# projecthorus/radiosonde_auto_rx

Measured on AMD Instinct MI355X. Metric: IQ Msamples/s (RS41 --IQ --lpIQ demod + framesync + ECC), concurrent real-time 2.4 Msps channels = value/2.4, higher is better.
Workload: dtype f32; 1 GPU; RS41 2.4 Msps cs16 IQ, rs41mod --ecc2 --IQ fq --lpIQ (BASELINE configs[1]) x 512 channels per GPU (per-GPU share of configs[4]), 1 s of signal per channel per step, input resident in HBM; channels_per_gpu=512, frames_decoded=507392, frames_ecc_ok=457842, frames_ecc_failed=49550, frames_repaired=200182, symbols_repaired=1815512

## Files before the change

radiosonde_auto_rx_amd/csrc/sonde_dev.h:

```cpp
#ifndef SONDE_DEV_H
#define SONDE_DEV_H
#include <hip/hip_runtime.h>
#include <stdint.h>
#include "../../include/sonde_hip.h"

struct MixDecArgs {
    const int16_t *iq;
    long long ch_stride;
    int n_ch, nblocks;
    int D, Q;
    int G;
    int wgs_per_ch;
    float wtab[64 * 8];
    const double *chan_f0;
    int lut_len;
    uint32_t lut_phase;
    const float2 *dc_avg;
    long long *dc_sums;
    const float2 *ptail_in;
    float2 *ptail_out;
    float2 *y;
    int ring_len;
    uint32_t m0;
    const float *wtab_g;
// ... 66 lines not shown
};

struct AudioChainArgs {
    const float *raw; float *fm, *bufs; const float *w;
    int n_ch, ring_len, n, taps; uint32_t m0;
};

struct SyncState {
    uint32_t s_in, k, mv_pos, mode;
    float mv; uint32_t inv;
    uint32_t pad[2];
};

struct WinItem {
    uint32_t pos;
    int32_t  state;
    int32_t  rc;
    float    mv; uint32_t mpos;
    uint32_t pad[3];
};
struct WinPlanArgs {
    const SyncState *state; WinItem *items;
    int n_ch, stride, W, K, L, delay; uint32_t frame_samples, avail;
    const uint32_t *epoch;
    uint32_t *work, *work_count; int round_parity;
};
struct WinFftArgs {
    const float *bufs; WinItem *items; const float2 *Fm, *tws;
    int n_ch, stride, W, K, L, ring_len;
    const uint32_t *work, *work_count; int round_parity;
    unsigned long long *prof;
    int small_wg;
    float2 *park;
};
#define SONDE_WFH_MAXGRID 768

struct CorrArgs {
    const float *bufs; float *corr; const float *match;
    const SyncState *state;
    const uint32_t *start;
    int delay; uint32_t frame_samples;
    uint32_t limit;
    int n_ch, ring_len, n, L; uint32_t m0;
    int ntypes, isps, nsym;
    const float *shapes;
    const int *sym_type;
    const float *sym_sign;
};

struct FrameRec {
    int32_t channel, len, nbytes; uint32_t mv_pos; float mv;
    int32_t ecc, ecc_done;
    uint8_t synd[48];
    uint8_t frame[520];
};

struct SyncArgs {
    const float *bufs, *corr; SyncState *state; FrameRec *frames; unsigned *frame_count; float *soft;
    float *soft1;
    const uint8_t *hdr, *hdr_bytes, *mask, *gf_exp, *gf_log;
    const uint4 *bitwin;
    const uint32_t *bitend;
    int n_ch, ring_len, max_frames; uint32_t avail;
    int K, L, delay, hdrlen, symhd, symlen, hdmax, bitofs, nbits; uint32_t frame_samples;
    float sps, thres, l_win;
    int rs41;
// ... 48 lines not shown
```

radiosonde_auto_rx_amd/csrc/sonde_engine.cpp:

```cpp
#include "../../include/sonde_hip.h"
#include "sonde_dev.h"
#include "sonde_host.h"
#include "sonde_scan_dev.h"
#include <algorithm>
#include <cmath>
#include <cstdio>
#include <cstring>
#include <map>
#include <string>
#include <vector>

using namespace sonde;

#define HIPCHK(x) do { hipError_t e_ = (x); if (e_ != hipSuccess) { fprintf(stderr, "libsonde_hip: %s failed: %s\n", #x, hipGetErrorString(e_)); return SONDE_E_NOGPU; } } while (0)

struct KernelStat { double ms = 0; int64_t n = 0; };
struct PendingEvt { hipEvent_t a, b; const char *name; };

struct sonde_engine {
    sonde_cfg_t cfg{};
    sonde_info_t info{};
    hipStream_t stream = nullptr;
    hipStream_t stream_b = nullptr;
    unsigned long long *d_wfprof = nullptr;
// ... 24 lines not shown
    float *d_wiq = nullptr, *d_wfm = nullptr, *d_match = nullptr;
    uint32_t corr_limit = 0;
    WinItem *d_win = nullptr; float2 *d_Fm = nullptr, *d_tws = nullptr; int win_W = 0;
    uint32_t *d_work = nullptr, *d_work_count = nullptr; int sync_rounds = 0;
    sonde_summary_t *d_summary = nullptr; uint32_t summary_base = 0;
    sonde_summary_t *d_summary_snap = nullptr;
    int corr_types = 0, corr_isps = 0; float *d_shapes = nullptr, *d_symsign = nullptr; int *d_symtype = nullptr;
    SyncState *d_state = nullptr; FrameRec *d_frames = nullptr; unsigned *d_fcount = nullptr; float *d_soft = nullptr, *d_soft1 = nullptr;
    uint4 *d_bitwin = nullptr; uint32_t *d_bitend = nullptr;
    uint8_t *d_consts = nullptr;
    int16_t *d_stage = nullptr; size_t stage_bytes = 0;
    bool ifiq = false;
    int opt_iq = 5; float match_sum = 0.f;
    std::vector<float> w_iq0; float *d_wiq0 = nullptr;
    float2 *d_yrot = nullptr; float *d_fmraw = nullptr, *d_corr2 = nullptr;
    AfcState *d_afc = nullptr; uint32_t *d_start = nullptr; unsigned *d_pending = nullptr, *h_pending = nullptr;
    double *d_dcsums_f = nullptr; float2 *d_zring = nullptr; float *d_taps_f = nullptr; uint32_t zmask = 0;
    hipEvent_t ev_copy = nullptr;
    int16_t *d_conv = nullptr;
    float2 *d_conv32 = nullptr; bool f32_path = false, conv32 = false;
    int ring_len = 0, max_frames = 0;
    uint64_t samples_in = 0;
    uint32_t m_out = 0;
    uint32_t dc_cnt = 0, dc_max = 0, dc_lim = 0;
    bool pcs = false; std::vector<uint32_t> pcs_cnt, pcs_max; uint32_t dc_max0 = 0;
    uint32_t *d_epoch_phase = nullptr, *d_pcs_cnt = nullptr, *d_pcs_max = nullptr; int32_t *d_pcs_since = nullptr;
    std::vector<float> last_soft, last_soft1; int last_n = 0;
    std::vector<uint8_t> last_frame;
    std::vector<char> m10_bits;
    bool overflow = false;
    bool in_call = false, ecc_listed = false;
    float2 *d_park = nullptr;
    bool small_tail = false;
    bool dev_ecc = true;
    long long host_ecc_frames = 0;
    bool m10_chk3 = false;
    std::vector<uint32_t> epoch; uint32_t *d_epoch = nullptr; int eof_ch = -1;
    bool prof = false, prof_skip = false; int prof_level = 2; std::map<std::string, KernelStat> stats; std::vector<PendingEvt> pend;
    std::vector<sonde_engine *> groups; std::vector<int32_t> grp_of_ch, row_of_ch; std::vector<std::vector<int32_t>> ch_of_grp; int32_t *d_in_row = nullptr;
    bool front_only = false; int64_t snap_calls = 0;
    sonde_engine *front = nullptr; int front_row = 0; int32_t *d_sum_map = nullptr; bool is_group = false;
    bool merged = false, borrowed_b = false;
};
struct CreateLink { bool is_group, front_only; int min_ring; hipStream_t shared_b; };

template <class T> static int dalloc(T **p, size_t n, bool zero = true) {
    HIPCHK(hipMalloc((void **)p, n * sizeof(T)));
    if (zero) HIPCHK(hipMemset(*p, 0, n * sizeof(T)));
    return 0;
}

static void prof_begin(sonde_engine *e, const char *name, hipStream_t s) {
    if (!e->prof || (e->prof_level == 1 && strcmp(name, "mix_decimate") != 0)) { e->prof_skip = true; return; }
    e->prof_skip = false;
    PendingEvt p; p.name = name;
    hipEventCreate(&p.a); hipEventCreate(&p.b);
    hipEventRecord(p.a, s);
    e->pend.push_back(p);
}
static void prof_end(sonde_engine *e, hipStream_t s) { if (e->prof && !e->prof_skip) hipEventRecord(e->pend.back().b, s); }
static void prof_collect(sonde_engine *e) {
    for (auto &p : e->pend) {
        float ms = 0; hipEventSynchronize(p.b); hipEventElapsedTime(&ms, p.a, p.b);
        auto &s = e->stats[p.name]; s.ms += ms; s.n += 1;
        hipEventDestroy(p.a); hipEventDestroy(p.b);
    }
// ... 289 lines not shown
        HIPCHK(hipMemcpy(e->d_chanf0, f0s.data(), f0s.size() * sizeof(double), hipMemcpyHostToDevice));
    }
    {
        static const bool no_fast = getenv("SONDE_MD_NOFAST") != nullptr;
        if (D == 50 && e->Q == 7 && !audio && cfg->bits != 32 && cfg->sonde_type != SONDE_FRONTEND && !cfg->opt_nolut && e->lut_len % D == 0 && !no_fast
            && cfg->input == SONDE_IN_IQ && !is_group) {
            e->etab_len = e->lut_len / D;
            if (dalloc(&e->d_etab, (size_t)C * e->etab_len, false) || dalloc(&e->d_dcavg_prev, C)) { sonde_engine_destroy(e); return SONDE_E_NOMEM; }
            sonde_launch_md_etable(e->d_chanf0, e->d_wtab, D, e->Q, e->etab_len, C, e->d_etab, nullptr);
            HIPCHK(hipDeviceSynchronize());
        }
    }
    int bad = 0;
    bad |= dalloc(&e->d_dcavg, C); bad |= dalloc(&e->d_dcsums, 2 * (size_t)C);
    bad |= dalloc(&e->d_ptail[0], (size_t)C * 64); bad |= dalloc(&e->d_ptail[1], (size_t)C * 64);
    if (audio) bad |= dalloc(&e->d_raw, (size_t)C * ring);
    else { if (!is_group) bad |= dalloc(&e->d_y, (size_t)C * ring); if (!front_only) bad |= dalloc(&e->d_ifiq, (size_t)C * ring); }
    if (!front_only) { bad |= dalloc(&e->d_fm, (size_t)C * ring); bad |= dalloc(&e->d_bufs, (size_t)C * ring); bad |= dalloc(&e->d_corr, (size_t)C * ring); }
    bad |= dalloc(&e->d_state, C); bad |= dalloc(&e->d_frames, e->max_frames); bad |= dalloc(&e->d_fcount, 1 + 4);
    if (cfg->keep_soft || cfg->sonde_type != SONDE_RS41) bad |= dalloc(&e->d_soft, (size_t)e->max_frames * e->nbits);
    if (cfg->keep_soft == 2) bad |= dalloc(&e->d_soft1, (size_t)e->max_frames * e->nbits);
    if (cfg->sonde_type == SONDE_DFM09) { bad |= dalloc(&e->d_dfm_out, (size_t)e->max_frames * 8); bad |= dalloc(&e->d_blk_done, 2); }
    if (cfg->sonde_type == SONDE_M10) { bad |= dalloc(&e->d_m10_out, (size_t)e->max_frames); bad |= dalloc(&e->d_blk_done, 2); bad |= dalloc(&e->d_m10_bits, (size_t)C * ((101 + 20) * 8 + 8)); }
    bad |= dalloc(&e->d_match, L, false);
    if (!e->w_iq.empty()) bad |= dalloc(&e->d_wiq, e->w_iq.size(), false);
    if (!e->w_fm.empty()) bad |= dalloc(&e->d_wfm, e->w_fm.size(), false);
    bad |= dalloc(&e->d_consts, 1024, true);
    if (bad) { sonde_engine_destroy(e); return SONDE_E_NOMEM; }
    HIPCHK(hipMemcpy(e->d_match, e->match.data(), L * sizeof(float), hipMemcpyHostToDevice));
    e->dev_ecc = getenv("SONDE_HOST_ECC") == nullptr;
    {
        const char *st = getenv("SONDE_SMALL_TAIL");
        e->small_tail = st && atoi(st) != 0;
    }
    {
        static const bool no_fft = getenv("SONDE_NO_FFTSYNC") != nullptr;
        if (!cfg->opt_dc && M == 8192 && K + L <= M && !no_fft) {
            std::vector<float> m(2 * (size_t)M, 0.f);
            for (int i = 0; i < L; i++) m[2 * (size_t)(L - 1 - i)] = e->match[i];
            ref_dft_8192(m);
            const std::vector<float> tw = ref_twiddle_table();
            e->win_W = 8;
            m.resize(4 * (size_t)M);
            for (int i = 0; i < M; i++) {
                int r = 0; for (int b = 0; b < 13; b++) if (i >> b & 1) r |= 1 << (12 - b);
                m[2 * (size_t)(M + i)] = m[2 * (size_t)r]; m[2 * (size_t)(M + i) + 1] = m[2 * (size_t)r + 1];
            }
            if (dalloc(&e->d_Fm, 2 * (size_t)M, false) || dalloc(&e->d_tws, tw.size() / 2, false) || dalloc(&e->d_win, (size_t)C * e->win_W) ||
                dalloc(&e->d_work, (size_t)C * e->win_W) || dalloc(&e->d_work_count, 2)) { sonde_engine_destroy(e); return SONDE_E_NOMEM; }
            HIPCHK(hipMemcpy(e->d_Fm, m.data(), m.size() * sizeof(float), hipMemcpyHostToDevice));
            HIPCHK(hipMemcpy(e->d_tws, tw.data(), tw.size() * sizeof(float), hipMemcpyHostToDevice));
        }
    }
    if (e->d_wiq) HIPCHK(hipMemcpy(e->d_wiq, e->w_iq.data(), e->w_iq.size() * sizeof(float), hipMemcpyHostToDevice));
    if (e->d_wfm) HIPCHK(hipMemcpy(e->d_wfm, e->w_fm.data(), e->w_fm.size() * sizeof(float), hipMemcpyHostToDevice));
    {
        uint8_t cb[1024]; memset(cb, 0, sizeof cb);
        memcpy(cb, header.data(), header.size()); memcpy(cb + 64, kRs41HeaderBytes, 8); memcpy(cb + 72, kRs41Mask, 64);
        memcpy(cb + 136, gf_exp_table(), 512); memcpy(cb + 648, gf_log_table(), 256);
        HIPCHK(hipMemcpy(e->d_consts, cb, sizeof cb, hipMemcpyHostToDevice));
    }
    {
        const int isps = (int)e->sps_design, nsym = e->hdrlen / e->symhd;
        if ((float)isps == e->sps_design && e->symhd == 1 && isps * nsym == L && isps >= 2 && isps <= 16 && isps % 2 == 0) {
            std::vector<float> shapes; std::vector<int> type(nsym); std::vector<float> sign(nsym);
            std::vector<int> key;
// ... 434 lines not shown

static int tail_finish(sonde_engine *e) {
    const int C = e->cfg.n_channels;
    const int slot = (int)(e->call & 3);
    hipStream_t se = e->stream_b;
    hipMemcpyAsync(e->d_fcount + 1 + slot, e->d_fcount, sizeof(unsigned), hipMemcpyDeviceToDevice, e->stream_b);
    if (e->ecc_listed) {
        if (e->stream_e) { hipEventRecord(e->ev_s, e->stream_b); hipStreamWaitEvent(e->stream_e, e->ev_s, 0); se = e->stream_e; }
        const int par = (int)(e->call & 1);
        prof_begin(e, "rs_ecc", se);
        sonde_launch_rs41_ecc_frames(e->d_frames, e->d_ecc_list + (size_t)par * e->max_frames, e->d_ecc_cnt + par, e->d_ecc_cnt + 2 + par, e->max_frames,
                                     e->cfg.ecc_level, e->d_consts + 136, e->d_consts + 648, std::min(512, std::max(1, C)), se);
        prof_end(e, se);
    }
    sonde_launch_publish_u32(e->d_fcount + 1 + slot, e->h_count_dev + slot, se);
    hipEventRecord(e->ev_b[slot], se);
    e->in_call = false;
    e->call += 1;
    if (hipPeekAtLastError() != hipSuccess) { fprintf(stderr, "libsonde_hip: launch failed: %s\n", hipGetErrorString(hipGetLastError())); return SONDE_E_NOGPU; }
    return 0;
}


extern "C" {

static void fill_round(sonde_engine *e, int W, WinPlanArgs &p, WinFftArgs &f) {
    const int C = e->cfg.n_channels;
    p = WinPlanArgs{}; p.state = e->d_state; p.items = e->d_win; p.n_ch = C; p.stride = e->win_W; p.W = W; p.K = e->info.K; p.L = e->info.L;
    p.delay = e->info.delay; p.frame_samples = e->frame_samples; p.avail = e->m_out; p.epoch = e->d_epoch;
    p.work = e->d_work; p.work_count = e->d_work_count; p.round_parity = e->sync_rounds & 1;
    f = WinFftArgs{}; f.bufs = e->d_bufs; f.items = e->d_win; f.Fm = e->d_Fm; f.tws = e->d_tws; f.n_ch = C; f.stride = e->win_W; f.W = W;
    f.K = e->info.K; f.L = e->info.L; f.ring_len = e->ring_len;
    f.work = e->d_work; f.work_count = e->d_work_count; f.round_parity = e->sync_rounds & 1; f.small_wg = e->small_tail; f.park = e->d_park;
    if (f.small_wg && !e->d_park) { if (hipMalloc((void **)&e->d_park, (size_t)SONDE_WFH_MAXGRID * 8192 * sizeof(float2)) != hipSuccess) f.small_wg = 0; f.park = e->d_park; }
    static const bool want_prof = getenv("SONDE_WF_PROF") != nullptr;
    if (want_prof && !e->d_wfprof) { if (hipMalloc((void **)&e->d_wfprof, 32 * sizeof(unsigned long long)) == hipSuccess) hipMemset(e->d_wfprof, 0, 32 * sizeof(unsigned long long)); }
    f.prof = e->d_wfprof;
    e->sync_rounds++;
}
static void sync_round(sonde_engine *e, int W) {
    hipStream_t sb = e->stream_b;
    WinPlanArgs p; WinFftArgs f;
    fill_round(e, W, p, f);
    prof_begin(e, "header_corr", sb);
    sonde_launch_sync_plan(&p, sb);
    sonde_launch_sync_window_fft(&f, sb);
    prof_end(e, sb);
    launch_framesync(e, 0);
}

static SyncArgs fill_sync(sonde_engine *e, int eof) {
    const int C = e->cfg.n_channels;
    SyncArgs s{};
    s.eof = eof; s.eof_ch = e->eof_ch; s.epoch = e->d_epoch; s.rs41 = (e->cfg.sonde_type == SONDE_RS41); s.ecc_level = (s.rs41 && e->dev_ecc && e->cfg.ecc_level >= 1 && e->cfg.ecc_level <= 2) ? e->cfg.ecc_level : 0;
    if (s.ecc_level && !eof && e->in_call && e->d_ecc_list) { s.ecc_list = e->d_ecc_list + (size_t)(e->call & 1) * e->max_frames; s.ecc_count = e->d_ecc_cnt + (e->call & 1); e->ecc_listed = true; }
    s.bufs = e->d_bufs; s.corr = e->d_corr; s.state = e->d_state; s.frames = e->d_frames; s.frame_count = e->d_fcount; s.soft = e->d_soft; s.soft1 = e->d_soft1;
    s.hdr = e->d_consts; s.hdr_bytes = e->d_consts + 64; s.mask = e->d_consts + 72; s.gf_exp = e->d_consts + 136; s.gf_log = e->d_consts + 648;
    s.bitwin = e->d_bitwin; s.bitend = e->d_bitend;
    s.small_wg = e->small_tail && !e->cfg.opt_dc;
    s.n_ch = C; s.ring_len = e->ring_len; s.max_frames = e->max_frames; s.avail = e->m_out;
    s.K = e->info.K; s.L = e->info.L; s.delay = e->info.delay; s.hdrlen = e->hdrlen; s.symhd = e->symhd; s.symlen = e->symlen;
    s.hdmax = e->hdmax; s.bitofs = e->bitofs; s.nbits = e->nbits; s.frame_samples = e->frame_samples;
    s.sps = e->sps; s.thres = e->thres; s.l_win = e->l_win;
    s.opt_auto = e->cfg.opt_auto != 0 || e->cfg.sonde_type == SONDE_M10 || e->cfg.sonde_type == SONDE_M20;
    s.opt_dc = e->cfg.opt_dc != 0; s.opt_iq = e->opt_iq; s.lpiq_on = !e->w_iq.empty(); s.lpfm_taps = (int)e->w_fm.size(); s.N = e->info.N; s.sr = e->info.if_sr;
    s.match_sum = e->match_sum; s.fm = e->d_fm; s.corr2 = e->d_corr2; s.ifiq = e->d_ifiq; s.afc = e->d_afc; s.start = e->d_start; s.pending = e->d_pending;
// ... 576 lines not shown
```

radiosonde_auto_rx_amd/csrc/sonde_fft_dev.h:

```cpp
#ifndef SONDE_FFT_DEV_H
#define SONDE_FFT_DEV_H
#include "sonde_scan_dev.h"
#ifndef FFT_THREADS
#define FFT_THREADS SC_THREADS
#endif

__device__ __forceinline__ float2 cmul(float2 a, float2 b) { return make_float2(a.x * b.x - a.y * b.y, a.x * b.y + a.y * b.x); }

#define XI(i) ((i) + ((i) >> 4) + ((i) >> 8))
#define SC_XN (SC_N + SC_N / 16 + SC_N / 256)

__device__ __forceinline__ int brev13(int k) { return (int)(__brev((unsigned)k) >> (32 - SC_LOG2N)); }

template <int R>
__device__ __forceinline__ void dit_pass(float2 *x, const float2 *tws, const int t0, const int tid) {
    constexpr int E = 1 << R;
    const int p_lo = t0;
#pragma unroll 1
    for (int g = tid; g < (SC_N >> R); g += FFT_THREADS) {
        const int low = g & ((1 << p_lo) - 1), high = g >> p_lo;
        const int base = (high << (p_lo + R)) | low;
        float2 v[E];
#pragma unroll
        for (int e = 0; e < E; e++) v[e] = x[XI(base + (e << p_lo))];
#pragma unroll
        for (int s = 0; s < R; s++) {
            const int t = t0 + s, bit = 1 << s;
#pragma unroll
            for (int e = 0; e < E; e++) {
                if (e & bit) continue;
                const int idx = base + (e << p_lo);
                const float2 w = tws[((1 << t) - 1) + (idx & ((1 << t) - 1))];
                const float2 p = v[e], r = cmul(v[e | bit], w);
                v[e] = make_float2(p.x + r.x, p.y + r.y);
                v[e | bit] = make_float2(p.x - r.x, p.y - r.y);
            }
        }
#pragma unroll
        for (int e = 0; e < E; e++) x[XI(base + (e << p_lo))] = v[e];
    }
    __syncthreads();
}

#define SC_TW_LDS 511
__device__ __forceinline__ void dft_ref_head(float2 *x, const float2 *tws, const float2 *tws_g, const int tid) {
    dit_pass<3>(x, tws, 0, tid);
    dit_pass<3>(x, tws, 3, tid);
    dit_pass<3>(x, tws, 6, tid);
    dit_pass<3>(x, tws_g, 9, tid);
}
__device__ __forceinline__ void dft_ref(float2 *x, const float2 *tws, const float2 *tws_g, const int tid) {
    dft_ref_head(x, tws, tws_g, tid);
    dit_pass<1>(x, tws_g, 12, tid);
}

#endif
```

radiosonde_auto_rx_amd/csrc/sonde_kernels.hip:

```cpp
#include <hip/hip_runtime.h>
#include <stdint.h>
#include "sonde_dev.h"
#include "md_fast_gen.h"
#include "sonde_rs_dev.h"
#include <cstdlib>

typedef short  short2v __attribute__((ext_vector_type(2)));

#define WAVE 64

#define MD_ROWS   64
#define MD_NVMAX  16

struct __attribute__((packed, aligned(4))) u32x4_u { uint32_t x, y, z, w; };

typedef float float2v __attribute__((ext_vector_type(2)));

__device__ __forceinline__ float2v cmul_pk(float2v u, float2v cs) {
    float2v t, z;
    asm("s_nop 0\n\tv_pk_mul_f32 %0, %1, %2 op_sel:[1,1] op_sel_hi:[1,0] neg_lo:[0,1]" : "=&v"(t) : "v"(u), "v"(cs));
    asm("v_pk_fma_f32 %0, %1, %2, %3 op_sel_hi:[0,1,1]" : "=&v"(z) : "v"(u), "v"(cs), "v"(t));
    return z;
}

// ... 1829 lines not shown
        for (int i = 0; i < n; i++) a.work[at + (uint32_t)i] = (uint32_t)(ch * a.stride + i);
    }
    if (a.work && first_thread) a.work_count[a.round_parity ^ 1] = 0;
    for (; n < a.stride; n++) { it[n].pos = 0xffffffffu; it[n].state = 0; }
}
__global__ void k_sync_plan(const WinPlanArgs a) {
    const int ch = blockIdx.x * blockDim.x + threadIdx.x;
    sync_plan_body(a, ch, ch == 0);
}
__global__ void k_sync_plan_multi(const MultiArgs<WinPlanArgs> m) {
    const int row = blockIdx.x * blockDim.x + threadIdx.x;
    if (row >= m.row0[m.n_groups]) return;
    int g = 0;
    while (g + 1 < m.n_groups && row >= m.row0[g + 1]) g++;
    sync_plan_body(m.g[g], row - m.row0[g], row == m.row0[g]);
}

#pragma clang fp contract(off)
#ifndef WF_THREADS
#define WF_THREADS 512
#endif
#define FFT_THREADS WF_THREADS
#include "sonde_fft_dev.h"
#ifndef WF_MB
#define WF_MB 4
#endif
#ifndef WF_LU
#define WF_LU 1
#endif
#ifndef WF_LB
#define WF_LB 4
#endif
#define WF_MARK(k) do { if (a.prof && blockIdx.x == 0 && tid == 0) { const unsigned long long t_ = __builtin_readcyclecounter(); a.prof[k] += t_ - t_prev; t_prev = t_; } } while (0)
__device__ __forceinline__ void sync_eval_window(const WinFftArgs &a, const int ch, WinItem *it, float2 *x, float2 *tws, float *s_rf, int *s_ri) {
    const int tid = threadIdx.x, lane = tid & 63, wave = tid >> 6;
    if (it->state != 1) return;
    unsigned long long t_prev = a.prof ? __builtin_readcyclecounter() : 0ull;
    const int K = a.K, L = a.L, N = SC_N, wl = K + L;
    const uint32_t pos = it->pos, mask = (uint32_t)a.ring_len - 1;
    const float *bufs = a.bufs + (size_t)ch * a.ring_len;
    const int64_t start = (int64_t)pos - (wl - 1);
    {
        constexpr int NL = SC_N / WF_THREADS;
#pragma unroll 1
        for (int h = 0; h < NL; h += WF_LB) {
            float v[WF_LB];
#pragma unroll
            for (int u = 0; u < WF_LB; u++) {
                const int i = tid + (h + u) * WF_THREADS;
                const int64_t p = start + i;
                v[u] = (i < wl && p >= 0) ? bufs[(uint32_t)p & mask] : 0.f;
            }
#pragma unroll
            for (int u = 0; u < WF_LB; u++) x[XI(brev13(tid + (h + u) * WF_THREADS))] = make_float2(v[u], 0.f);
        }
    }
    __syncthreads();
    WF_MARK(0);
    dft_ref(x, tws, a.tws, tid);
    WF_MARK(1);
    {
        const float2 *FmR = a.Fm + N;
#pragma unroll 1
        for (int h = 0; h < N / WF_THREADS; h += WF_MB) {
            float2 fi[WF_MB], fr[WF_MB];
#pragma unroll
            for (int u = 0; u < WF_MB; u++) {
                const int i = tid + (h + u) * WF_THREADS;
                const bool on = brev13(i) >= i;
                fi[u] = on ? a.Fm[i] : make_float2(0.f, 0.f);
                fr[u] = on ? FmR[i] : make_float2(0.f, 0.f);
            }
#pragma unroll
            for (int u = 0; u < WF_MB; u++) {
                const int i = tid + (h + u) * WF_THREADS, r = brev13(i);
                if (r < i) continue;
                const float2 zi = cmul(x[XI(i)], fi[u]), zr = cmul(x[XI(r)], fr[u]);
                x[XI(r)] = make_float2(zi.x, -zi.y);
                x[XI(i)] = make_float2(zr.x, -zr.y);
            }
        }
    }
    __syncthreads();
    WF_MARK(2);
    dft_ref_head(x, tws, a.tws, tid);
    float best = 0.f, bestc = 0.f; int bidx = -1;
#pragma unroll WF_LU
    for (int u = 0; u < SC_N / 2 / WF_THREADS; u++) {
        const int g = tid + u * WF_THREADS;
        const float2 w = a.tws[((1 << 12) - 1) + g];
        const float2 p = x[XI(g)], r = cmul(x[XI(g + (1 << 12))], w);
        const float c0 = p.x + r.x, c1 = p.x - r.x;
        const int i0 = g, i1 = g + (1 << 12);
        if (i0 >= L - 1 && i0 < wl) { const float c2 = c0 * c0; if (c2 > best || (c2 == best && bidx >= 0 && i0 < bidx)) { best = c2; bidx = i0; bestc = c0; } }
        if (i1 >= L - 1 && i1 < wl) { const float c2 = c1 * c1; if (c2 > best || (c2 == best && bidx >= 0 && i1 < bidx)) { best = c2; bidx = i1; bestc = c1; } }
    }
    WF_MARK(3);
    {
        float rb = best; int ri = bidx;
        for (int off = 32; off > 0; off >>= 1) {
            const float ob = __shfl_xor(rb, off); const int oi = __shfl_xor(ri, off);
            if (ob > rb || (ob == rb && oi >= 0 && (ri < 0 || oi < ri))) { rb = ob; ri = oi; }
        }
        if (lane == 0) { s_rf[wave] = rb; s_ri[wave] = ri; }
    }
    __syncthreads();
    int mp = -1;
    {
        float b = 0.f;
        for (int w = 0; w < WF_THREADS / WAVE; w++) {
            const float ob = s_rf[w]; const int oi = s_ri[w];
            if (ob > b || (ob == b && oi >= 0 && (mp < 0 || oi < mp))) { b = ob; mp = oi; }
        }
    }
    __syncthreads();
    WF_MARK(4);
    if (mp < 0) {
        if (tid == 0) { it->rc = -5; it->mv = 0.f; it->mpos = pos - (uint32_t)(wl - 1) - 1u; __threadfence(); it->state = 2; }
        return;
    }
    if (mp == L - 1 || mp == wl - 1) {
        if (tid == 0) { it->rc = -4; it->mv = 0.f; it->mpos = 0; __threadfence(); it->state = 2; }
        return;
    }
    float e = 0.f;
    for (int k = tid; k < L; k += WF_THREADS) {
        const int i = mp - k; const int64_t p2 = start + i;
        const float v = (i < wl && p2 >= 0) ? bufs[(uint32_t)p2 & mask] : 0.f;
        e += v * v;
    }
    for (int off = 32; off > 0; off >>= 1) e += __shfl_xor(e, off);
    if (lane == 0) s_rf[wave] = e;
    if (bidx == mp) s_rf[WF_THREADS / WAVE] = bestc;
    __syncthreads();
    if (tid == 0) {
        float es = 0.f;
        for (int w = 0; w < WF_THREADS / WAVE; w++) es += s_rf[w];
        const float xnorm = sqrtf(es);
        it->rc = mp; it->mv = s_rf[WF_THREADS / WAVE] / (xnorm * (float)N); it->mpos = pos - (uint32_t)(wl - 1) + (uint32_t)mp;
        __threadfence(); it->state = 2;
    }
    WF_MARK(5);
    if (a.prof && blockIdx.x == 0 && tid == 0) a.prof[15] += 1;
}

#if WF_THREADS <= 512
#define WF_WAVES_ATTR __attribute__((amdgpu_waves_per_eu(2 * WF_THREADS / 256, 2 * WF_THREADS / 256)))
#else
#define WF_WAVES_ATTR
#endif
__device__ __forceinline__ void sync_window_fft_body(const WinFftArgs &a, const uint32_t b, const uint32_t nb) {
    extern __shared__ __attribute__((aligned(16))) float2 smem2[];
    float2 *x = smem2;
    float2 *tws = smem2 + SC_XN;
    __shared__ float s_rf[WF_THREADS / WAVE + 1];
    __shared__ int s_ri[WF_THREADS / WAVE];
    const uint32_t count = a.work_count[a.round_parity];
    if (b >= count) return;
    for (int k = threadIdx.x; k < SC_TW_LDS; k += WF_THREADS) tws[k] = a.tws[k];
    for (uint32_t w = b; w < count; w += nb) {
        const uint32_t item = a.work[w];
        __syncthreads();
        sync_eval_window(a, (int)(item / (uint32_t)a.stride), a.items + item, x, tws, s_rf, s_ri);
    }
}
__global__ __launch_bounds__(WF_THREADS) WF_WAVES_ATTR
void k_sync_window_fft(const WinFftArgs a) { sync_window_fft_body(a, blockIdx.x, gridDim.x); }
__global__ __launch_bounds__(WF_THREADS) WF_WAVES_ATTR
void k_sync_window_fft_multi(const MultiArgs<WinFftArgs> m) {
    const int g = multi_group(m, (int)blockIdx.x);
    sync_window_fft_body(m.g[g], blockIdx.x - (uint32_t)m.row0[g], (uint32_t)(m.row0[g + 1] - m.row0[g]));
}
#define WFH_THREADS 256
#define SCH_N (SC_N / 2)
#define SCH_XN (SCH_N + SCH_N / 16 + SCH_N / 256)
template <int R>
__device__ __forceinline__ void dit_pass_h(float2 *x, const float2 *tws, const int t0, const int tid) {
    constexpr int E = 1 << R;
    const int p_lo = t0;
#pragma unroll 1
    for (int g = tid; g < (SCH_N >> R); g += WFH_THREADS) {
        const int low = g & ((1 << p_lo) - 1), high = g >> p_lo;
        const int base = (high << (p_lo + R)) | low;
        float2 v[E];
#pragma unroll
        for (int e = 0; e < E; e++) v[e] = x[XI(base + (e << p_lo))];
#pragma unroll
        for (int s2 = 0; s2 < R; s2++) {
            const int t = t0 + s2, bit = 1 << s2;
#pragma unroll
            for (int e = 0; e < E; e++) {
                if (e & bit) continue;
                const int idx = base + (e << p_lo);
                const float2 w = tws[((1 << t) - 1) + (idx & ((1 << t) - 1))];
                const float2 p = v[e], r = cmul(v[e | bit], w);
                v[e] = make_float2(p.x + r.x, p.y + r.y);
                v[e | bit] = make_float2(p.x - r.x, p.y - r.y);
            }
        }
#pragma unroll
        for (int e = 0; e < E; e++) x[XI(base + (e << p_lo))] = v[e];
    }
    __syncthreads();
}
// ... 320 lines not shown
    return m;
}
extern "C" int sonde_launch_if_chain_multi(const IfArgs *a, int n_groups, hipStream_t s) {
    if (n_groups < 1 || n_groups > SONDE_MAX_GROUPS) return -1;
    size_t lds = 0; int rows[SONDE_MAX_GROUPS], n = a[0].n;
    for (int g = 0; g < n_groups; g++) {
        const int T1 = a[g].lpiq_on ? a[g].lpiq_taps : 1, T2 = a[g].lpfm_on ? a[g].lpfm_taps : 1;
        const int hz = (T2 - 1) + (a[g].nwin - 1 > 1 ? a[g].nwin - 1 : 1);
        const int nz = hz + IF_TILE, ny = nz + T1 - 1;
        const size_t l = (size_t)((ny + 2 * IF_NB + 1) & ~1) * 8 + (size_t)(a[g].fm_on ? nz + 1 : 0) * 8 + (size_t)(a[g].tone_on ? nz : 0) * 16 + (size_t)(a[g].fm_on ? T2 - 1 + IF_TILE : 0) * 4 + (size_t)(T1 + T2) * 4 + 32;
        if (l > lds) lds = l;
        rows[g] = a[g].n_ch;
        if (a[g].n != n) return -1;
    }
    const MultiArgs<IfArgs> m = multi_pack(a, rows, n_groups);
    hipLaunchKernelGGL(k_if_chain_multi, dim3((n + IF_TILE - 1) / IF_TILE, m.row0[n_groups]), dim3(IF_THREADS), lds, s, m);
    return 0;
}
extern "C" int sonde_launch_sync_plan_multi(const WinPlanArgs *a, int n_groups, hipStream_t s) {
    if (n_groups < 1 || n_groups > SONDE_MAX_GROUPS) return -1;
    int rows[SONDE_MAX_GROUPS];
    for (int g = 0; g < n_groups; g++) rows[g] = a[g].n_ch;
    const MultiArgs<WinPlanArgs> m = multi_pack(a, rows, n_groups);
    hipLaunchKernelGGL(k_sync_plan_multi, dim3((m.row0[n_groups] + 255) / 256), dim3(256), 0, s, m);
    return 0;
}
extern "C" int sonde_launch_sync_window_fft_multi(const WinFftArgs *a, int n_groups, hipStream_t s) {
    if (n_groups < 1 || n_groups > SONDE_MAX_GROUPS) return -1;
    long long tot = 0; int rows[SONDE_MAX_GROUPS];
    for (int g = 0; g < n_groups; g++) tot += (long long)a[g].W * a[g].n_ch;
    const long long cap = tot > 512 ? 512 : tot;
    for (int g = 0; g < n_groups; g++) { const long long w = (long long)a[g].W * a[g].n_ch; rows[g] = (int)((w * cap + tot - 1) / tot); if (rows[g] < 1) rows[g] = 1; }
    const MultiArgs<WinFftArgs> m = multi_pack(a, rows, n_groups);
    hipLaunchKernelGGL(k_sync_window_fft_multi, dim3(m.row0[n_groups]), dim3(WF_THREADS), (size_t)(SC_XN + SC_TW_LDS + 1) * sizeof(float2), s, m);
    return 0;
}
extern "C" void sonde_launch_header_corr(const CorrArgs *a, hipStream_t s) {
    if (a->ntypes > 0) {
        const int nf = (HCF_TILE + a->isps * (a->nsym - 1) + 3) & ~3, nxp = (nf + a->isps + 3 + 3) & ~3;
        const size_t lds = (size_t)(nxp + a->ntypes * nf) * sizeof(float);
        hipLaunchKernelGGL(k_header_corr_fact, dim3((a->n + HCF_TILE - 1) / HCF_TILE, a->n_ch), dim3(HCF_THREADS), lds, s, *a);
        return;
    }
    const size_t lds = (size_t)(HC_TILE + 2 * a->L + 8) * sizeof(float);
    hipLaunchKernelGGL(k_header_corr, dim3((a->n + HC_TILE - 1) / HC_TILE, a->n_ch), dim3(HC_THREADS), lds, s, *a);
}
extern "C" void sonde_launch_sync_plan(const WinPlanArgs *a, hipStream_t s) {
    hipLaunchKernelGGL(k_sync_plan, dim3((a->n_ch + 255) / 256), dim3(256), 0, s, *a);
}
extern "C" void sonde_launch_sync_window_fft(const WinFftArgs *a, hipStream_t s) {
    const size_t lds = (size_t)(SC_XN + SC_TW_LDS + 1) * sizeof(float2);
    int grid = a->W * a->n_ch;
    if (a->small_wg) {
        if (grid > SONDE_WFH_MAXGRID) grid = SONDE_WFH_MAXGRID;
        hipLaunchKernelGGL(k_sync_window_fft_h, dim3(grid), dim3(WFH_THREADS), (size_t)(SCH_XN + SC_TW_LDS + 1) * sizeof(float2), s, *a);
        return;
    }
    if (grid > 512) grid = 512;
    hipLaunchKernelGGL(k_sync_window_fft, dim3(grid), dim3(WF_THREADS), lds, s, *a);
}
#define RSK_THREADS 256
struct RsEccLds { uint8_t frame[520], exp[512], log[256], cw[2][256], part[RSK_THREADS / 64][48], scr[2][64], S[48]; int res[4]; };
__device__ __forceinline__ void rs_ecc_tables(RsEccLds &L, const uint8_t *gf_exp, const uint8_t *gf_log, int tid) {
    for (int i = tid; i < 512; i += RSK_THREADS) L.exp[i] = gf_exp[i];
    if (tid < 256) L.log[tid] = gf_log[tid];
}
__global__ __launch_bounds__(RSK_THREADS)
void k_rs41_ecc_frames(FrameRec *frames, const uint32_t *list, unsigned *count, unsigned *done, int max_frames, int level,
                       const uint8_t *gf_exp, const uint8_t *gf_log) {
    __shared__ RsEccLds L;
    __shared__ unsigned s_last;
    const int tid = threadIdx.x;
    const unsigned n = min(*count, (unsigned)max_frames);
    if (n) rs_ecc_tables(L, gf_exp, gf_log, tid);
    for (unsigned w = blockIdx.x; w < n; w += gridDim.x) {
        FrameRec *rec = frames + list[w];
        __syncthreads();
        if (rec->ecc_done != 2) continue;
        const int flen = rec->len;
        for (int i = tid; i < 518; i += RSK_THREADS) L.frame[i] = i < flen ? rec->frame[i] : 0;
        if (tid < 48) L.S[tid] = rec->synd[tid];
        __syncthreads();
        const RsGf gf{L.exp, L.log};
        const int r = rs41_ecc_wg(L.frame, level, L.cw, L.part, L.res, L.scr, L.S, gf, tid, RSK_THREADS);
        for (int i = tid; i < 518; i += RSK_THREADS) rec->frame[i] = L.frame[i];
        __threadfence();
        __syncthreads();
        if (tid == 0) { rec->ecc = r; rec->ecc_done = 1; }
    }
    __syncthreads();
    if (tid == 0) { __threadfence(); s_last = atomicAdd(done, 1u); }
    __syncthreads();
// ... 49 lines not shown
```

Baseline: 873,700 Msamples/s.

## Use register-resident radix-16 FFT for sync window correlation by default

Adds a new sync-window FFT kernel in which each thread keeps 16 elements in registers and runs radix-16 DIT stages, with only the transposes between stages going through LDS. A padded index map avoids LDS bank conflicts. The matched-filter spectrum and last-stage twiddles stay in registers, and the new kernel becomes the default, with the old LDS form kept behind SONDE_WF_LDS. The aim is fewer LDS round trips and barriers per FFT, paid for with higher register pressure and possibly lower occupancy.

```diff
diff --git a/radiosonde_auto_rx_amd/csrc/sonde_dev.h b/radiosonde_auto_rx_amd/csrc/sonde_dev.h
--- a/radiosonde_auto_rx_amd/csrc/sonde_dev.h
+++ b/radiosonde_auto_rx_amd/csrc/sonde_dev.h
@@ -122,6 +122,7 @@
     unsigned long long *prof;
     int small_wg;
     float2 *park;
+    int lds_form;
 };
 #define SONDE_WFH_MAXGRID 768
 
diff --git a/radiosonde_auto_rx_amd/csrc/sonde_engine.cpp b/radiosonde_auto_rx_amd/csrc/sonde_engine.cpp
--- a/radiosonde_auto_rx_amd/csrc/sonde_engine.cpp
+++ b/radiosonde_auto_rx_amd/csrc/sonde_engine.cpp
@@ -80,6 +80,7 @@
     bool in_call = false, ecc_listed = false;
     float2 *d_park = nullptr;
     bool small_tail = false;
+    bool wf_lds = false;
     bool dev_ecc = true;
     long long host_ecc_frames = 0;
     bool m10_chk3 = false;
@@ -435,6 +436,8 @@
     {
         const char *st = getenv("SONDE_SMALL_TAIL");
         e->small_tail = st && atoi(st) != 0;
+        const char *wl = getenv("SONDE_WF_LDS");
+        e->wf_lds = wl && atoi(wl) != 0;
     }
     {
         static const bool no_fft = getenv("SONDE_NO_FFTSYNC") != nullptr;
@@ -935,6 +938,7 @@
     f = WinFftArgs{}; f.bufs = e->d_bufs; f.items = e->d_win; f.Fm = e->d_Fm; f.tws = e->d_tws; f.n_ch = C; f.stride = e->win_W; f.W = W;
     f.K = e->info.K; f.L = e->info.L; f.ring_len = e->ring_len;
     f.work = e->d_work; f.work_count = e->d_work_count; f.round_parity = e->sync_rounds & 1; f.small_wg = e->small_tail; f.park = e->d_park;
+    f.lds_form = e->wf_lds;
     if (f.small_wg && !e->d_park) { if (hipMalloc((void **)&e->d_park, (size_t)SONDE_WFH_MAXGRID * 8192 * sizeof(float2)) != hipSuccess) f.small_wg = 0; f.park = e->d_park; }
     static const bool want_prof = getenv("SONDE_WF_PROF") != nullptr;
     if (want_prof && !e->d_wfprof) { if (hipMalloc((void **)&e->d_wfprof, 32 * sizeof(unsigned long long)) == hipSuccess) hipMemset(e->d_wfprof, 0, 32 * sizeof(unsigned long long)); }
diff --git a/radiosonde_auto_rx_amd/csrc/sonde_fft_dev.h b/radiosonde_auto_rx_amd/csrc/sonde_fft_dev.h
--- a/radiosonde_auto_rx_amd/csrc/sonde_fft_dev.h
+++ b/radiosonde_auto_rx_amd/csrc/sonde_fft_dev.h
@@ -54,4 +54,42 @@
     dit_pass<1>(x, tws_g, 12, tid);
 }
 
+#define XJ(i) ((i) + ((i) >> 5) + ((i) >> 9))
+#define SC_XJN (SC_N + SC_N / 32 + SC_N / 512)
+#define SC_TWJ_LDS 1023
+__device__ __forceinline__ int brev9(int k) { return (int)(__brev((unsigned)k) >> 23); }
+__host__ __device__ constexpr int brev4(int e) { return ((e & 1) << 3) | ((e & 2) << 1) | ((e & 4) >> 1) | ((e & 8) >> 3); }
+__device__ __forceinline__ int dit16_base(const int t0, const int tid) { return ((tid >> t0) << (t0 + 4)) | (tid & ((1 << t0) - 1)); }
+__host__ __device__ constexpr int xj_off(const int t0, const int e) { return t0 == 0 ? e : t0 == 4 ? 16 * e + (e >> 1) : 264 * e + (e >> 1); }
+#define XJ_U 529
+template <int T0>
+__device__ __forceinline__ void dit16_regs(float2 *v, const float2 *tws, const float2 *tws_g, const int lo) {
+    const float2 *twl = tws + lo, *twg = tws_g + lo;
+#pragma unroll
+    for (int s = 0; s < 4; s++) {
+        const int t = T0 + s, bit = 1 << s;
+#pragma unroll
+        for (int e = 0; e < 16; e++) {
+            if (e & bit) continue;
+            const float2 w = (t <= 9 ? twl : twg)[((1 << t) - 1) + ((e & (bit - 1)) << T0)];
+            const float2 p = v[e], r = cmul(v[e | bit], w);
+            v[e] = make_float2(p.x + r.x, p.y + r.y);
+            v[e | bit] = make_float2(p.x - r.x, p.y - r.y);
+        }
+    }
+}
+__device__ __forceinline__ int dit16_opaque(int v) { asm volatile("" : "+v"(v)); return v; }
+template <int T0>
+__device__ __forceinline__ void dit16_pass(float2 *x, const float2 *tws, const float2 *tws_g, int tid) {
+    tid = dit16_opaque(tid);
+    float2 *xb = x + XJ(dit16_base(T0, tid));
+    float2 v[16];
+#pragma unroll
+    for (int e = 0; e < 16; e++) v[e] = xb[xj_off(T0, e)];
+    dit16_regs<T0>(v, tws, tws_g, tid & ((1 << T0) - 1));
+#pragma unroll
+    for (int e = 0; e < 16; e++) xb[xj_off(T0, e)] = v[e];
+    __syncthreads();
+}
+
 #endif
diff --git a/radiosonde_auto_rx_amd/csrc/sonde_kernels.hip b/radiosonde_auto_rx_amd/csrc/sonde_kernels.hip
--- a/radiosonde_auto_rx_amd/csrc/sonde_kernels.hip
+++ b/radiosonde_auto_rx_amd/csrc/sonde_kernels.hip
@@ -1885,8 +1885,60 @@
 #define WF_LB 4
 #endif
 #define WF_MARK(k) do { if (a.prof && blockIdx.x == 0 && tid == 0) { const unsigned long long t_ = __builtin_readcyclecounter(); a.prof[k] += t_ - t_prev; t_prev = t_; } } while (0)
+__device__ __forceinline__ void sync_window_finish(const WinFftArgs &a, WinItem *it, const float *bufs, const uint32_t pos, const int64_t start, const int wl,
+                                                   const float best, const float bestc, const int bidx, float *s_rf, int *s_ri, unsigned long long &t_prev) {
+    const int tid = threadIdx.x, lane = tid & 63, wave = tid >> 6;
+    const int L = a.L, N = SC_N;
+    const uint32_t mask = (uint32_t)a.ring_len - 1;
+    {
+        float rb = best; int ri = bidx;
+        for (int off = 32; off > 0; off >>= 1) {
+            const float ob = __shfl_xor(rb, off); const int oi = __shfl_xor(ri, off);
+            if (ob > rb || (ob == rb && oi >= 0 && (ri < 0 || oi < ri))) { rb = ob; ri = oi; }
+        }
+        if (lane == 0) { s_rf[wave] = rb; s_ri[wave] = ri; }
+    }
+    __syncthreads();
+    int mp = -1;
+    {
+        float b = 0.f;
+        for (int w = 0; w < WF_THREADS / WAVE; w++) {
+            const float ob = s_rf[w]; const int oi = s_ri[w];
+            if (ob > b || (ob == b && oi >= 0 && (mp < 0 || oi < mp))) { b = ob; mp = oi; }
+        }
+    }
+    __syncthreads();
+    WF_MARK(4);
+    if (mp < 0) {
+        if (tid == 0) { it->rc = -5; it->mv = 0.f; it->mpos = pos - (uint32_t)(wl - 1) - 1u; __threadfence(); it->state = 2; }
+        return;
+    }
+    if (mp == L - 1 || mp == wl - 1) {
+        if (tid == 0) { it->rc = -4; it->mv = 0.f; it->mpos = 0; __threadfence(); it->state = 2; }
+        return;
+    }
+    float e = 0.f;
+    for (int k = tid; k < L; k += WF_THREADS) {
+        const int i = mp - k; const int64_t p2 = start + i;
+        const float v = (i < wl && p2 >= 0) ? bufs[(uint32_t)p2 & mask] : 0.f;
+        e += v * v;
+    }
+    for (int off = 32; off > 0; off >>= 1) e += __shfl_xor(e, off);
+    if (lane == 0) s_rf[wave] = e;
+    if (bidx == mp) s_rf[WF_THREADS / WAVE] = bestc;
+    __syncthreads();
+    if (tid == 0) {
+        float es = 0.f;
+        for (int w = 0; w < WF_THREADS / WAVE; w++) es += s_rf[w];
+        const float xnorm = sqrtf(es);
+        it->rc = mp; it->mv = s_rf[WF_THREADS / WAVE] / (xnorm * (float)N); it->mpos = pos - (uint32_t)(wl - 1) + (uint32_t)mp;
+        __threadfence(); it->state = 2;
+    }
+    WF_MARK(5);
+    if (a.prof && blockIdx.x == 0 && tid == 0) a.prof[15] += 1;
+}
 __device__ __forceinline__ void sync_eval_window(const WinFftArgs &a, const int ch, WinItem *it, float2 *x, float2 *tws, float *s_rf, int *s_ri) {
-    const int tid = threadIdx.x, lane = tid & 63, wave = tid >> 6;
+    const int tid = threadIdx.x;
     if (it->state != 1) return;
     unsigned long long t_prev = a.prof ? __builtin_readcyclecounter() : 0ull;
     const int K = a.K, L = a.L, N = SC_N, wl = K + L;
@@ -1949,52 +2001,7 @@
         if (i1 >= L - 1 && i1 < wl) { const float c2 = c1 * c1; if (c2 > best || (c2 == best && bidx >= 0 && i1 < bidx)) { best = c2; bidx = i1; bestc = c1; } }
     }
     WF_MARK(3);
-    {
-        float rb = best; int ri = bidx;
-        for (int off = 32; off > 0; off >>= 1) {
-            const float ob = __shfl_xor(rb, off); const int oi = __shfl_xor(ri, off);
-            if (ob > rb || (ob == rb && oi >= 0 && (ri < 0 || oi < ri))) { rb = ob; ri = oi; }
-        }
-        if (lane == 0) { s_rf[wave] = rb; s_ri[wave] = ri; }
-    }
-    __syncthreads();
-    int mp = -1;
-    {
-        float b = 0.f;
-        for (int w = 0; w < WF_THREADS / WAVE; w++) {
-            const float ob = s_rf[w]; const int oi = s_ri[w];
-            if (ob > b || (ob == b && oi >= 0 && (mp < 0 || oi < mp))) { b = ob; mp = oi; }
-        }
-    }
-    __syncthreads();
-    WF_MARK(4);
-    if (mp < 0) {
-        if (tid == 0) { it->rc = -5; it->mv = 0.f; it->mpos = pos - (uint32_t)(wl - 1) - 1u; __threadfence(); it->state = 2; }
-        return;
-    }
-    if (mp == L - 1 || mp == wl - 1) {
-        if (tid == 0) { it->rc = -4; it->mv = 0.f; it->mpos = 0; __threadfence(); it->state = 2; }
-        return;
-    }
-    float e = 0.f;
-    for (int k = tid; k < L; k += WF_THREADS) {
-        const int i = mp - k; const int64_t p2 = start + i;
-        const float v = (i < wl && p2 >= 0) ? bufs[(uint32_t)p2 & mask] : 0.f;
-        e += v * v;
-    }
-    for (int off = 32; off > 0; off >>= 1) e += __shfl_xor(e, off);
-    if (lane == 0) s_rf[wave] = e;
-    if (bidx == mp) s_rf[WF_THREADS / WAVE] = bestc;
-    __syncthreads();
-    if (tid == 0) {
-        float es = 0.f;
-        for (int w = 0; w < WF_THREADS / WAVE; w++) es += s_rf[w];
-        const float xnorm = sqrtf(es);
-        it->rc = mp; it->mv = s_rf[WF_THREADS / WAVE] / (xnorm * (float)N); it->mpos = pos - (uint32_t)(wl - 1) + (uint32_t)mp;
-        __threadfence(); it->state = 2;
-    }
-    WF_MARK(5);
-    if (a.prof && blockIdx.x == 0 && tid == 0) a.prof[15] += 1;
+    sync_window_finish(a, it, bufs, pos, start, wl, best, bestc, bidx, s_rf, s_ri, t_prev);
 }
 
 #if WF_THREADS <= 512
@@ -2023,6 +2030,90 @@
 void k_sync_window_fft_multi(const MultiArgs<WinFftArgs> m) {
     const int g = multi_group(m, (int)blockIdx.x);
     sync_window_fft_body(m.g[g], blockIdx.x - (uint32_t)m.row0[g], (uint32_t)(m.row0[g + 1] - m.row0[g]));
+}
+static_assert(WF_THREADS * 16 == SC_N, "the register-resident form holds 16 elements per thread");
+__device__ __forceinline__ void sync_eval_window_r(const WinFftArgs &a, const int ch, WinItem *it, float2 *x, const float2 *tws, const float2 *fm, const float2 *w12,
+                                                   float *s_rf, int *s_ri) {
+    const int tid = threadIdx.x;
+    if (it->state != 1) return;
+    unsigned long long t_prev = a.prof ? __builtin_readcyclecounter() : 0ull;
+    const int K = a.K, L = a.L, wl = K + L;
+    const uint32_t pos = it->pos, mask = (uint32_t)a.ring_len - 1;
+    const float *bufs = a.bufs + (size_t)ch * a.ring_len;
+    const int64_t start = (int64_t)pos - (wl - 1);
+    float2 *const x0 = x + XJ(brev9(tid) << 4);
+    float2 *const xn = x + XJ(tid);
+    float2 v[16];
+    const int tl = dit16_opaque(tid);
+#pragma unroll
+    for (int e = 0; e < 16; e++) {
+        const int i = tl + WF_THREADS * brev4(e);
+        const int64_t p = start + i;
+        v[e] = make_float2((i < wl && p >= 0) ? bufs[(uint32_t)p & mask] : 0.f, 0.f);
+    }
+    dit16_regs<0>(v, tws, a.tws, 0);
+#pragma unroll
+    for (int e = 0; e < 16; e++) x0[e] = v[e];
+    __syncthreads();
+    WF_MARK(0);
+    dit16_pass<4>(x, tws, a.tws, tid);
+    dit16_pass<8>(x, tws, a.tws, tid);
+    WF_MARK(1);
+#pragma unroll
+    for (int u = 0; u < 8; u++) {
+        const float2 p = xn[XJ_U * u], r = cmul(xn[XJ_U * (u + 8)], w12[u]);
+        const float2 z0 = cmul(make_float2(p.x + r.x, p.y + r.y), fm[u]), z1 = cmul(make_float2(p.x - r.x, p.y - r.y), fm[u + 8]);
+        v[brev4(u)] = make_float2(z0.x, -z0.y);
+        v[brev4(u + 8)] = make_float2(z1.x, -z1.y);
+    }
+    __syncthreads();
+    WF_MARK(2);
+    dit16_regs<0>(v, tws, a.tws, 0);
+#pragma unroll
+    for (int e = 0; e < 16; e++) x0[e] = v[e];
+    __syncthreads();
+    dit16_pass<4>(x, tws, a.tws, tid);
+    dit16_pass<8>(x, tws, a.tws, tid);
+    float best = 0.f, bestc = 0.f; int bidx = -1;
+#pragma unroll
+    for (int u = 0; u < 8; u++) {
+        const int g = tid + WF_THREADS * u;
+        const float2 p = xn[XJ_U * u], r = cmul(xn[XJ_U * (u + 8)], w12[u]);
+        const float c0 = p.x + r.x, c1 = p.x - r.x;
+        const int i0 = g, i1 = g + (1 << 12);
+        if (i0 >= L - 1 && i0 < wl) { const float c2 = c0 * c0; if (c2 > best || (c2 == best && bidx >= 0 && i0 < bidx)) { best = c2; bidx = i0; bestc = c0; } }
+        if (i1 >= L - 1 && i1 < wl) { const float c2 = c1 * c1; if (c2 > best || (c2 == best && bidx >= 0 && i1 < bidx)) { best = c2; bidx = i1; bestc = c1; } }
+    }
+    WF_MARK(3);
+    sync_window_finish(a, it, bufs, pos, start, wl, best, bestc, bidx, s_rf, s_ri, t_prev);
+}
+__device__ __forceinline__ void sync_window_fft_r_body(const WinFftArgs &a, const uint32_t b, const uint32_t nb) {
+    extern __shared__ __attribute__((aligned(16))) float2 smem2[];
+    float2 *x = smem2;
+    float2 *tws = smem2 + SC_XJN;
+    __shared__ float s_rf[WF_THREADS / WAVE + 1];
+    __shared__ int s_ri[WF_THREADS / WAVE];
+    const uint32_t count = a.work_count[a.round_parity];
+    if (b >= count) return;
+    const int tid = threadIdx.x;
+    for (int k = tid; k < SC_TWJ_LDS; k += WF_THREADS) tws[k] = a.tws[k];
+    float2 fm[16], w12[8];
+#pragma unroll
+    for (int u = 0; u < 16; u++) fm[u] = a.Fm[tid + WF_THREADS * u];
+#pragma unroll
+    for (int u = 0; u < 8; u++) w12[u] = a.tws[((1 << 12) - 1) + tid + WF_THREADS * u];
+    for (uint32_t w = b; w < count; w += nb) {
+        const uint32_t item = a.work[w];
+        __syncthreads();
+        sync_eval_window_r(a, (int)(item / (uint32_t)a.stride), a.items + item, x, tws, fm, w12, s_rf, s_ri);
+    }
+}
+__global__ __launch_bounds__(WF_THREADS) WF_WAVES_ATTR
+void k_sync_window_fft_r(const WinFftArgs a) { sync_window_fft_r_body(a, blockIdx.x, gridDim.x); }
+__global__ __launch_bounds__(WF_THREADS) WF_WAVES_ATTR
+void k_sync_window_fft_r_multi(const MultiArgs<WinFftArgs> m) {
+    const int g = multi_group(m, (int)blockIdx.x);
+    sync_window_fft_r_body(m.g[g], blockIdx.x - (uint32_t)m.row0[g], (uint32_t)(m.row0[g + 1] - m.row0[g]));
 }
 #define WFH_THREADS 256
 #define SCH_N (SC_N / 2)
@@ -2409,7 +2500,8 @@
     const long long cap = tot > 512 ? 512 : tot;
     for (int g = 0; g < n_groups; g++) { const long long w = (long long)a[g].W * a[g].n_ch; rows[g] = (int)((w * cap + tot - 1) / tot); if (rows[g] < 1) rows[g] = 1; }
     const MultiArgs<WinFftArgs> m = multi_pack(a, rows, n_groups);
-    hipLaunchKernelGGL(k_sync_window_fft_multi, dim3(m.row0[n_groups]), dim3(WF_THREADS), (size_t)(SC_XN + SC_TW_LDS + 1) * sizeof(float2), s, m);
+    if (a[0].lds_form) hipLaunchKernelGGL(k_sync_window_fft_multi, dim3(m.row0[n_groups]), dim3(WF_THREADS), (size_t)(SC_XN + SC_TW_LDS + 1) * sizeof(float2), s, m);
+    else hipLaunchKernelGGL(k_sync_window_fft_r_multi, dim3(m.row0[n_groups]), dim3(WF_THREADS), (size_t)(SC_XJN + SC_TWJ_LDS + 1) * sizeof(float2), s, m);
     return 0;
 }
 extern "C" void sonde_launch_header_corr(const CorrArgs *a, hipStream_t s) {
@@ -2434,7 +2526,8 @@
         return;
     }
     if (grid > 512) grid = 512;
-    hipLaunchKernelGGL(k_sync_window_fft, dim3(grid), dim3(WF_THREADS), lds, s, *a);
+    if (a->lds_form) hipLaunchKernelGGL(k_sync_window_fft, dim3(grid), dim3(WF_THREADS), lds, s, *a);
+    else hipLaunchKernelGGL(k_sync_window_fft_r, dim3(grid), dim3(WF_THREADS), (size_t)(SC_XJN + SC_TWJ_LDS + 1) * sizeof(float2), s, *a);
 }
 #define RSK_THREADS 256
 struct RsEccLds { uint8_t frame[520], exp[512], log[256], cw[2][256], part[RSK_THREADS / 64][48], scr[2][64], S[48]; int res[4]; };
```

After: 888,100 Msamples/s, median of 6. No clear change (+1.6%).
